# SAR-Research-Lab/lvt

Measured on AMD Instinct MI355X. Metric: stereo frames/sec (KITTI-shaped 1241x376), per-frame SE3 vs CPU ref, higher is better.
Workload: dtype u8/f64

## Files before the change

### include/lvt_amd_ext.h

```cpp
#ifndef LVT_AMD_EXT_H__
#define LVT_AMD_EXT_H__

#include "lvt_c.h"
#include <stdint.h>

#ifdef __cplusplus
extern "C" {
#endif

typedef struct lvt_amd_params {
    float fx, fy, cx, cy;
    float baseline;
    int img_width, img_height;
    float k1, k2, p1, p2, k3;
    float near_plane_distance, far_plane_distance;
    float triangulation_ratio_test_threshold;
    float tracking_ratio_test_threshold;
    float descriptor_matching_threshold;
    int min_num_matches_for_tracking;
    int tracking_radius;
    int detection_cell_size;
    int max_keypoints_per_cell;
    int agast_threshold;
    int untracked_threshold;
// ... 43 lines not shown
                                       unsigned *score, int score_cap, int counts[2]);

LVT_API void lvt_amd_set_stream(lvt_handle h, void *hip_stream);
LVT_API const char *lvt_amd_last_error(lvt_handle h);

LVT_API void lvt_amd_get_host_stats(lvt_handle h, long long out[8]);

LVT_API void lvt_amd_profile_enable(lvt_handle h, int enable);
LVT_API int lvt_amd_profile_read(lvt_handle h, int slot, char *name, int name_cap, double *total_ms, long *calls);

enum {
    LVT_AMD_C_N_LEFT = 0, LVT_AMD_C_N_RIGHT, LVT_AMD_C_MAP_SIZE, LVT_AMD_C_STAGED_SIZE, LVT_AMD_C_N_MATCHES,
    LVT_AMD_C_SECOND_PASS, LVT_AMD_C_N_ROW_MATCHES, LVT_AMD_C_N_TRIANGULATED, LVT_AMD_C_TRIANGULATED,
    LVT_AMD_C_RETRY_LEFT, LVT_AMD_C_RETRY_RIGHT, LVT_AMD_C_PNP_ITERS, LVT_AMD_C_PNP_INLIERS,
    LVT_AMD_C_MAP_SIZE_AT_MATCH, LVT_AMD_C_N_STAGED_ERASED, LVT_AMD_C_N_STAGED_PROMOTED, LVT_AMD_C_N_CULLED,
    LVT_AMD_C_FRAME, LVT_AMD_C_OVERFLOW ,
    LVT_AMD_C_PNP_BORDERLINE ,
    LVT_AMD_C_ROW_FALLBACK ,
    LVT_AMD_C_PNP_TRIALS , LVT_AMD_C_PNP_REJECTIONS ,
    LVT_AMD_C_PNP_TERMINATES ,
    LVT_AMD_C__COUNT = 32
};
LVT_API void lvt_amd_get_counts(lvt_handle h, int out[LVT_AMD_C__COUNT]);
LVT_API int lvt_amd_get_features(lvt_handle h, int eye, float *xy, float *resp, uint8_t *desc, int cap);
LVT_API int lvt_amd_get_matches(lvt_handle h, int *feat_idx, double *xyz, int cap);
LVT_API int lvt_amd_get_row_matches(lvt_handle h, int *pairs, int cap);
LVT_API int lvt_amd_get_map(lvt_handle h, double *xyz, int *counter, int *age, uint8_t *desc, int cap);
LVT_API int lvt_amd_get_staged(lvt_handle h, double *xyz, int *counter, uint8_t *desc, int cap);
LVT_API void lvt_amd_get_pose(lvt_handle h, double q_wxyz[4], double p[3]);
LVT_API int lvt_amd_get_last_pose(lvt_handle h, double q_wxyz[4], double p[3]);
LVT_API void lvt_amd_get_predicted_pose(lvt_handle h, double q_wxyz[4], double p[3]);
LVT_API void lvt_amd_get_debug(lvt_handle h, long long out[32]);
LVT_API void lvt_amd_get_timeline(lvt_handle h, long long out[16]);
LVT_API int lvt_amd_get_ordering(lvt_handle h);
LVT_API int lvt_amd_get_plane(lvt_handle h, int eye, int what, void *dst, int cap_bytes, int *pitch_out);

LVT_API int lvt_amd_pnp(const lvt_amd_params *p, const double q_in[4], const double p_in[3], const double *pts,
                        const float *obs, int n, double q_out[4], double p_out[3], int *n_solve_calls);
LVT_API int lvt_amd_pnp_detail(const lvt_amd_params *p, const double q_in[4], const double p_in[3], const double *pts,
                               const float *obs, int n, double q_out[4], double p_out[3], int *n_solve_calls,
                               double *err_out, int *level_out, int *borderline);
LVT_API int lvt_amd_pnp_trace(const lvt_amd_params *p, const double q_in[4], const double p_in[3], const double *pts,
                              const float *obs, int n, double q_out[4], double p_out[3], int *n_solve_calls,
                              double *err_out, int *level_out, int *borderline, double *trace, int trace_cap, int stats[3]);
LVT_API int lvt_amd_motion_predict(double state[14], const double q[4], const double p[3], double q_out[4], double p_out[3]);
LVT_API float lvt_amd_hamming_match_batched(const void *q_desc, const void *q_xy, const void *t_desc,
                                            const void *t_xy, const void *t_flag, int B, int M, int N,
                                            float r2, int mode, int img_rows, int img_cols, void *out,
                                            void *hip_stream);
LVT_API float lvt_amd_hamming_match_batched_n(const void *q_desc, const void *q_xy, const void *t_desc,
                                              const void *t_xy, const void *t_flag, int B, int M, int N,
                                              float r2, int mode, int img_rows, int img_cols, void *out,
                                              void *hip_stream, int launches);

typedef void *lvt_amd_rectifier;
LVT_API lvt_amd_rectifier lvt_amd_rectifier_create(const double K[9], const double D[5], const double R[9],
                                                   const double Pnew[9], int width, int height);
LVT_API void lvt_amd_rectifier_destroy(lvt_amd_rectifier r);
LVT_API int lvt_amd_rectify_device(lvt_amd_rectifier r, const void *d_src, int src_pitch, void *d_dst, int dst_pitch,
                                   void *hip_stream);
LVT_API int lvt_amd_rectify(lvt_amd_rectifier r, const unsigned char *src, unsigned char *dst);
LVT_API int lvt_amd_rectifier_get_maps(lvt_amd_rectifier r, float *map1, float *map2);
LVT_API int lvt_amd_set_rectifiers(lvt_handle h, lvt_amd_rectifier left, lvt_amd_rectifier right);
LVT_API int lvt_amd_batch_set_rectifiers(lvt_handle h, int seq, lvt_amd_rectifier left, lvt_amd_rectifier right);

enum { LVT_AMD_PIX_GRAY8 = 0, LVT_AMD_PIX_BGR8 = 1, LVT_AMD_PIX_RGB8 = 2, LVT_AMD_PIX_BGRA8 = 3, LVT_AMD_PIX_RGBA8 = 4 };
// ... 18 lines not shown
```

### lvt_amd/__init__.py

```python
from __future__ import annotations

import ctypes as C
import os

import numpy as np

from .params import LvtParameters, ParamsPOD, kitti_params, euroc_params, tum_params

_HERE = os.path.dirname(os.path.abspath(__file__))
LIB_PATH = os.environ.get("LVT_AMD_LIB") or os.path.join(_HERE, "lib", "liblvt_c.so")

ABI_SYMBOLS = [
    "lvt_create", "lvt_destroy", "lvt_track", "lvt_track_with_external_corners", "lvt_get_status",
    "lvt_amd_default_params", "lvt_amd_params_from_file", "lvt_amd_create", "lvt_amd_reset",
    "lvt_amd_track_rgbd", "lvt_amd_track_device", "lvt_amd_track_device_async", "lvt_amd_wait",
    "lvt_amd_set_stream", "lvt_amd_last_error", "lvt_amd_get_counts", "lvt_amd_get_features",
    "lvt_amd_get_matches", "lvt_amd_get_row_matches", "lvt_amd_get_map", "lvt_amd_get_staged",
    "lvt_amd_get_pose", "lvt_amd_get_last_pose", "lvt_amd_get_predicted_pose", "lvt_amd_get_plane", "lvt_amd_pnp", "lvt_amd_pnp_detail",
    "lvt_amd_hamming_match_batched", "lvt_amd_hamming_match_batched_n", "lvt_amd_rectifier_create", "lvt_amd_rectifier_destroy",
    "lvt_amd_rectify_device", "lvt_amd_rectify", "lvt_amd_rectifier_get_maps",
    "lvt_amd_odometry_create", "lvt_amd_odometry_destroy", "lvt_amd_odometry_reset", "lvt_amd_odometry_push_pose", "lvt_amd_odometry_update", "lvt_amd_profile_enable", "lvt_amd_profile_read", "lvt_amd_get_debug", "lvt_amd_get_timeline", "lvt_amd_get_ordering",
    "lvt_amd_batch_create", "lvt_amd_batch_size", "lvt_amd_batch_track_device_async", "lvt_amd_batch_wait",
    "lvt_amd_batch_get_counts", "lvt_amd_create_on_device", "lvt_amd_get_device", "lvt_amd_wait_status", "lvt_amd_get_host_stats",
    "lvt_amd_track_async", "lvt_amd_track_rgbd_async", "lvt_amd_pnp_trace", "lvt_amd_create_pooled", "lvt_amd_wait_pose",
    "lvt_amd_batch_create_mixed", "lvt_amd_batch_track_device_async_mixed", "lvt_amd_batch_get_params", "lvt_amd_batch_mixed_tables",
    "lvt_amd_track_rgbd_device", "lvt_amd_track_rgbd_device_async", "lvt_amd_track_rgbd16", "lvt_amd_track_rgbd16_async",
    "lvt_amd_batch_track_rgbd_device_async",
    "lvt_amd_set_rectifiers", "lvt_amd_batch_set_rectifiers",
    "lvt_amd_set_pixel_format", "lvt_amd_batch_set_pixel_format", "lvt_amd_get_pixel_format",
    "lvt_amd_motion_predict",
]

N_COUNTS = 32
COUNT_NAMES = ["n_left", "n_right", "map_size", "staged_size", "n_matches", "second_pass", "n_row_matches",
               "n_triangulated", "triangulated", "retry_left", "retry_right", "pnp_iters", "pnp_inliers",
               "map_size_at_match", "n_staged_erased", "n_staged_promoted", "n_culled", "frame", "overflow", "pnp_borderline", "row_fallback", "pnp_trials", "pnp_rejections", "pnp_terminates"]

eState_NOT_INITIALIZED, eState_TRACKING, eState_LOST = 1, 2, 3
eSensor_STEREO, eSensor_RGBD = 1, 2
PIX_GRAY8, PIX_BGR8, PIX_RGB8, PIX_BGRA8, PIX_RGBA8 = 0, 1, 2, 3, 4
PIX_BPP = {PIX_GRAY8: 1, PIX_BGR8: 3, PIX_RGB8: 3, PIX_BGRA8: 4, PIX_RGBA8: 4}
DEPTH_F32, DEPTH_U16 = 0, 1

_lib = None


def load_library():
    global _lib
    if _lib is not None:
        return _lib
    if not os.path.exists(LIB_PATH):
        raise RuntimeError(f"{LIB_PATH} is missing: build it with `make -C lvt_amd/csrc` "
                           "(there is no CPU fallback for the tracking path)")
    try:
        import torch
    except Exception:
        pass
    L = C.CDLL(LIB_PATH)
    vp = C.c_void_p
    L.lvt_create.restype = vp
    L.lvt_create.argtypes = [C.c_char_p, C.c_int]
    L.lvt_amd_create.restype = vp
    L.lvt_amd_create.argtypes = [vp, C.c_int]
# ... 12 lines not shown
    L.lvt_amd_track_rgbd.argtypes = [vp, vp, vp, C.c_int, C.c_int, vp, vp]
    L.lvt_amd_track_device.argtypes = [vp, vp, vp, C.c_int, C.c_int, C.c_int, vp, vp]
    L.lvt_amd_track_device_async.argtypes = [vp, vp, vp, C.c_int, C.c_int, C.c_int]
    L.lvt_amd_wait.argtypes = [vp, vp, vp]
    L.lvt_amd_track_async.argtypes = [vp, vp, vp, C.c_int, C.c_int]
    L.lvt_amd_track_async.restype = C.c_int
    L.lvt_amd_track_rgbd_async.argtypes = [vp, vp, vp, C.c_int, C.c_int]
    L.lvt_amd_track_rgbd_async.restype = C.c_int
    L.lvt_amd_wait_status.argtypes = [vp, vp, vp]
    L.lvt_amd_wait_status.restype = C.c_int
    L.lvt_amd_set_stream.argtypes = [vp, vp]
    L.lvt_amd_last_error.restype = C.c_char_p
    L.lvt_amd_last_error.argtypes = [vp]
    L.lvt_amd_get_counts.argtypes = [vp, vp]
    L.lvt_amd_get_features.argtypes = [vp, C.c_int, vp, vp, vp, C.c_int]
    L.lvt_amd_get_matches.argtypes = [vp, vp, vp, C.c_int]
    L.lvt_amd_get_row_matches.argtypes = [vp, vp, C.c_int]
    L.lvt_amd_get_map.argtypes = [vp, vp, vp, vp, vp, C.c_int]
    L.lvt_amd_get_staged.argtypes = [vp, vp, vp, vp, C.c_int]
    L.lvt_amd_get_pose.argtypes = [vp, vp, vp]
    L.lvt_amd_get_last_pose.argtypes = [vp, vp, vp]
    L.lvt_amd_get_predicted_pose.argtypes = [vp, vp, vp]
    L.lvt_amd_get_plane.argtypes = [vp, C.c_int, C.c_int, vp, C.c_int, vp]
    L.lvt_amd_pnp.argtypes = [vp, vp, vp, vp, vp, C.c_int, vp, vp, vp]
    L.lvt_amd_pnp_detail.argtypes = [vp, vp, vp, vp, vp, C.c_int, vp, vp, vp, vp, vp, vp]
    L.lvt_amd_pnp_trace.argtypes = [vp, vp, vp, vp, vp, C.c_int, vp, vp, vp, vp, vp, vp, vp, C.c_int, vp]
    L.lvt_amd_motion_predict.argtypes = [vp, vp, vp, vp, vp]
    L.lvt_amd_motion_predict.restype = C.c_int
    L.lvt_amd_hamming_match_batched.restype = C.c_float
    L.lvt_amd_hamming_match_batched.argtypes = [vp, vp, vp, vp, vp, C.c_int, C.c_int, C.c_int, C.c_float, C.c_int, C.c_int, C.c_int, vp, vp]
    L.lvt_amd_get_timeline.argtypes = [vp, vp]
    L.lvt_amd_get_ordering.argtypes = [vp]
    L.lvt_amd_get_ordering.restype = C.c_int
    L.lvt_amd_rectifier_create.restype = vp
    L.lvt_amd_rectifier_create.argtypes = [vp, vp, vp, vp, C.c_int, C.c_int]
    L.lvt_amd_rectifier_destroy.argtypes = [vp]
    L.lvt_amd_rectify_device.argtypes = [vp, vp, C.c_int, vp, C.c_int, vp]
    L.lvt_amd_rectify.argtypes = [vp, vp, vp]
    L.lvt_amd_rectifier_get_maps.argtypes = [vp, vp, vp]
    L.lvt_amd_odometry_create.restype = vp
    L.lvt_amd_odometry_create.argtypes = [vp, vp, C.c_int]
    L.lvt_amd_odometry_destroy.argtypes = [vp]
    L.lvt_amd_odometry_reset.argtypes = [vp]
    L.lvt_amd_odometry_push_pose.restype = C.c_int
    L.lvt_amd_odometry_push_pose.argtypes = [vp, vp, vp, C.c_int, C.c_double, vp, vp]
    L.lvt_amd_odometry_update.restype = C.c_int
    L.lvt_amd_odometry_update.argtypes = [vp, vp, vp, C.c_int, C.c_int, C.c_double, vp, vp]
    L.lvt_amd_hamming_match_batched_n.restype = C.c_float
    L.lvt_amd_hamming_match_batched_n.argtypes = [vp, vp, vp, vp, vp, C.c_int, C.c_int, C.c_int, C.c_float, C.c_int, C.c_int, C.c_int, vp, vp, C.c_int]
    L.lvt_amd_profile_enable.argtypes = [vp, C.c_int]
    L.lvt_amd_batch_create.restype = vp
    L.lvt_amd_batch_create.argtypes = [vp, C.c_int, C.c_int]
    L.lvt_amd_batch_size.argtypes = [vp]
    L.lvt_amd_batch_track_device_async.argtypes = [vp, vp, vp, C.c_int, C.c_int, C.c_int]
    L.lvt_amd_batch_wait.argtypes = [vp, vp, vp, vp]
    L.lvt_amd_batch_get_counts.argtypes = [vp, C.c_int, vp]
    L.lvt_amd_batch_create_mixed.restype = vp
    L.lvt_amd_batch_create_mixed.argtypes = [vp, C.c_int, C.c_int]
    L.lvt_amd_batch_track_device_async_mixed.restype = C.c_int
    L.lvt_amd_batch_track_device_async_mixed.argtypes = [vp, vp, vp, vp, vp, vp]
    L.lvt_amd_batch_get_params.restype = C.c_int
    L.lvt_amd_batch_get_params.argtypes = [vp, C.c_int, vp]
    L.lvt_amd_batch_mixed_tables.restype = C.c_int
    L.lvt_amd_batch_mixed_tables.argtypes = [vp, C.c_int, C.c_int, vp, C.c_int, vp, C.c_int, vp]
    L.lvt_amd_batch_size.restype = C.c_int
    for name, argtypes in (
# ... 515 lines not shown
```

### lvt_amd/csrc/k_track.hip

```cpp
#include "lvt_dev.h"
#include "wave_reduce.h"
#include "lvt_math.h"

namespace lvt {

enum : int { MODE_MAP = 0, MODE_STAGED = 1, MODE_ROW = 2 };

__device__ __forceinline__ void frame_prologue(const Seq &S, Ctl &c, int par, const Pose &predicted, const double mm_next[14], bool active,
                                               bool first, bool skipped) {
    const bool absent = skipped && S.fb[par].fc->absent != 0;
    if (!absent) {
        for (int i = 0; i < N_COUNTS; i++) c.counts[i] = 0;
        c.counts[C_FRAME] = c.frame_number;
        c.frame_number++;
    }
    c.active = active ? 1 : 0;
    c.first_frame = first ? 1 : 0;
    c.do_pass2 = 0;
    c.n_pass1 = c.n_pass2 = 0;
    c.n_matches = 0;
    c.lost_now = 0;
    c.need_tri = 0;
    c.dont_stage = 0;
    c.n_pairs = 0;
// ... 250 lines not shown
            for (int e = lane; e < cnt; e += 64) {
                const uint32_t k = buf[e];
                int rank = 0;
                for (int o = 0; o < cnt; o++) rank += (buf[o] < k) ? 1 : 0;
                cand[(size_t)i * KC + rank] = k;
            }
        }
        if (lane == 0) ncand[i] = cnt;
        __builtin_amdgcn_fence(__ATOMIC_ACQ_REL, "workgroup");
    }
}

template <int MODE, bool BV>
__global__ __launch_bounds__(256) void k_candidates(SeqArg<BV> sa, int pass2, int par, seq_t need_seq, int only_fb) {
    const Seq &S = sa.get();
    if (only_fb && !S.lists_fb[MODE == MODE_ROW ? 1 : 0]) return;
    if (MODE != MODE_ROW) {
        const Ctl &ctl = *S.ctl;
        if (!ctl.active || ctl.first_frame) return;
        if (MODE == MODE_STAGED && (ctl.lost_now || S.prm.staged_th <= 0)) return;
    } else {
        if (S.prm.sensor != 1) return;
        if (need_seq && __hip_atomic_load(&S.fb[par].fc->feat_seq, __ATOMIC_ACQUIRE, __HIP_MEMORY_SCOPE_AGENT) < need_seq) return;
    }
    __shared__ uint32_t lbuf[4 * KC];
    __shared__ float s_tx[NF_MAX], s_ty[NF_MAX];
    __shared__ uint32_t s_tc[NF_MAX];
    CandLds C;
    C.lbuf = lbuf, C.tx = s_tx, C.ty = s_ty, C.tc = s_tc;
    candidates_body<MODE>(S, pass2, par, C, blockIdx.x * 4 + wave_id(), gridDim.x * 4, 256);
}

__device__ __forceinline__ void deliver_record(const Ctl &ctl, Ctl *rec_out, seq_t *done_out, seq_t seq, int nthreads);
__device__ __forceinline__ void gate_late_poll(Ctl &ctl, FeatCtl &fc, seq_t seq);
template <bool BV>
__global__ __launch_bounds__(256) void k_match_map(SeqArg<BV> sa, int par, seq_t seq, int gated, Ctl *prev_rec, seq_t *prev_done) {
    const Seq &S = sa.get();
    Ctl &ctl = *S.ctl;
    __shared__ int s_state;
    if (gated) {
        if (threadIdx.x == 0 && blockIdx.x == 0) ctl.dbg[38] = (long long)wall_clock64();
        if (blockIdx.x == 0 && prev_rec) deliver_record(ctl, prev_rec, prev_done, seq - 1, 256);
        if (threadIdx.x == 0) {
            if (blockIdx.x == 0) {
                gate_late_poll(ctl, *S.fb[par].fc, seq);
                __hip_atomic_store(&ctl.late_gate_seq, seq, __ATOMIC_RELEASE, __HIP_MEMORY_SCOPE_AGENT);
            } else {
                while (__hip_atomic_load(&ctl.late_gate_seq, __ATOMIC_ACQUIRE, __HIP_MEMORY_SCOPE_AGENT) < seq) __builtin_amdgcn_s_sleep(8);
            }
        }
    }
    if (threadIdx.x == 0 && blockIdx.x == 0) ctl.dbg[40] = (long long)wall_clock64();
    __shared__ int s_skip;
    if (threadIdx.x == 0) {
        int sk = ctl.skip;
        if (!gated && __hip_atomic_load(&S.fb[par].fc->skip_seq, __ATOMIC_ACQUIRE, __HIP_MEMORY_SCOPE_AGENT) == seq) {
            sk = 1;
            if (blockIdx.x == 0) ctl.skip = 1;
        }
        s_state = ctl.state, s_skip = sk;
    }
    __syncthreads();
    const int state = s_state;
    const bool skipped = s_skip != 0;
    const bool active = (state != 3) && !skipped, first = (state == 1);
    __shared__ double w2c[12];
    if (threadIdx.x == 0) {
        Pose predicted;
        double mmn[14];
        if (active && !first) {
            motion_predict(ctl, ctl.last_pose, predicted, mmn);
            world_to_camera(predicted, w2c);
        }
        if (blockIdx.x == 0) {
            frame_prologue(S, ctl, par, predicted, mmn, active, first, skipped);
            if (active && !first) ctl.counts[C_MAP_SIZE_AT_MATCH] = *S.map_n;
        }
    }
    if (!active || first) return;
    __shared__ uint32_t lbuf[4 * KC];
    __shared__ float s_tx[NF_MAX], s_ty[NF_MAX];
    __shared__ uint32_t s_tc[NF_MAX];
    CandLds C;
    C.lbuf = lbuf, C.tx = s_tx, C.ty = s_ty, C.tc = s_tc, C.w2c = w2c;
    candidates_body<MODE_MAP, true>(S, 0, par, C, blockIdx.x * 4 + wave_id(), gridDim.x * 4, 256, (ctl.early_ran_seq == seq) ? max(ctl.early_done, 0) : 0, -1);
}

__device__ __forceinline__ void gate_buf_wait(const Seq &S, seq_t want, int par) {
    Ctl &ctl = *S.ctl;
    const unsigned long long t0 = wall_clock64();
    while (__hip_atomic_load(&ctl.track_done_seq, __ATOMIC_ACQUIRE, __HIP_MEMORY_SCOPE_AGENT) < want) {
        __builtin_amdgcn_s_sleep(8);
        if (wall_clock64() - t0 > 200000000ull) {
            S.fb[par].fc->poison = 1;
            atomicAdd(&ctl.gate_fatal, 1);
            __threadfence();
            break;
        }
    }
}
__global__ __launch_bounds__(64) void k_gate_buf(const Seq *seqs, seq_t want, int par) {
    if (threadIdx.x != 0) return;
    gate_buf_wait(seq_const(seqs, blockIdx.z), want, par);
}

__global__ void k_feat_done(const Seq *seqs, int par, seq_t seq) {
    if (threadIdx.x != 0) return;
    FeatCtl &fc = *seq_const(seqs, blockIdx.x).fb[par].fc;
    seq_const(seqs, blockIdx.x).ctl->dbg[47] = (long long)wall_clock64();
    if (fc.poison) {
        fc.skip_seq = seq;
        fc.poison = 0;
    }
    __threadfence();
    atomicExch(&fc.feat_seq, seq);
}

__global__ void k_row_done(const Seq *seqs, int par, seq_t seq) {
    if (threadIdx.x != 0) return;
    FeatCtl &fc = *seq_const(seqs, blockIdx.x).fb[par].fc;
    if (__hip_atomic_load(&fc.feat_seq, __ATOMIC_ACQUIRE, __HIP_MEMORY_SCOPE_AGENT) < seq) return;
    __threadfence();
    atomicExch(&fc.row_seq, seq);
}

template <bool BV>
__global__ __launch_bounds__(64) void k_gate(SeqArg<BV> sa, int par, seq_t want, seq_t seq, int test_timeout) {
    if (threadIdx.x == 0 && blockIdx.x == 0) sa.get().ctl->dbg[32] = (long long)wall_clock64();
    Ctl &ctl = *sa.get().ctl;
    FeatCtl &fc = *sa.get().fb[par].fc;
    if (threadIdx.x != 0) return;
    bool ok = true;
    if (test_timeout) {
        atomicAdd(&ctl.gate_timeouts, 1);
        ok = false;
    } else {
        const unsigned long long t0 = wall_clock64();
        while (__hip_atomic_load(&fc.feat_seq, __ATOMIC_ACQUIRE, __HIP_MEMORY_SCOPE_AGENT) < seq) {
            __builtin_amdgcn_s_sleep(8);
            if (wall_clock64() - t0 > 2000000ull) {
                atomicAdd(&ctl.gate_timeouts, 1);
                ok = false;
                break;
            }
        }
        if (ok && __hip_atomic_load(&fc.skip_seq, __ATOMIC_ACQUIRE, __HIP_MEMORY_SCOPE_AGENT) == seq) ok = false;
        const unsigned long long t1 = wall_clock64();
        ctl.dbg[35] = (long long)t1;
        while (ok && __hip_atomic_load(&ctl.pnp_seq, __ATOMIC_ACQUIRE, __HIP_MEMORY_SCOPE_AGENT) < want) {
            __builtin_amdgcn_s_sleep(8);
            if (wall_clock64() - t1 > 2000000ull) {
                atomicAdd(&ctl.gate_timeouts, 1);
                ok = false;
                break;
            }
        }
    }
    const seq_t mine = 4u * seq + (ok ? 1u : 3u);
    seq_t cur = __hip_atomic_load(&ctl.early_state, __ATOMIC_ACQUIRE, __HIP_MEMORY_SCOPE_AGENT);
    for (;;) {
        if (cur >= 4u * seq + 1u) {
            ok = false;
            break;
        }
        const seq_t seen = atomicCAS(&ctl.early_state, cur, mine);
        if (seen == cur) break;
        cur = seen;
    }
    ctl.gate_ok = ok ? seq : (seq_t)0;
    ctl.dbg[33] = (long long)wall_clock64();
}

template <bool BV>
__global__ __launch_bounds__(256) void k_early_map(SeqArg<BV> sa, int par, seq_t seq, int only_fb) {
    if (threadIdx.x == 0 && blockIdx.x == 0) sa.get().ctl->dbg[34] = (long long)wall_clock64();
    const Seq &S = sa.get();
    if (only_fb && !S.lists_fb[0]) return;
    Ctl &ctl = *S.ctl;
    const int n_early = (ctl.gate_ok == seq) ? ctl.early_done : 0;
    if (n_early <= 0) return;
    __shared__ double w2c[12];
    if (threadIdx.x == 0) {
        Pose predicted;
        double mmn[14];
        motion_predict(ctl, ctl.last_pose, predicted, mmn);
        world_to_camera(predicted, w2c);
    }
    __shared__ uint32_t lbuf[4 * KC];
    __shared__ float s_tx[NF_MAX], s_ty[NF_MAX];
// ... 629 lines not shown
        {
            CandLds C;
            C.lbuf = r_lists;
            C.tx = reinterpret_cast<float *>(r_lists + 16 * KC);
            C.ty = C.tx + NF_MAX;
            C.tc = reinterpret_cast<uint32_t *>(C.ty + NF_MAX);
            candidates_body<MODE_MAP>(S, 1, par, C, wave_id(), RES_THREADS / 64, RES_THREADS);
        }
        __syncthreads();
        resolve_body<MODE_MAP>(S, ctl, 1, par, L, r_tab);
        __syncthreads();
    }
    if (*S.map_n <= RES_THREADS) {
        bookkeep_cull_small(S, ctl, par, L.scan);
        return;
    }
    bookkeep_cull_large(S, ctl, par, L.scan, L.lists);
}

template <bool BV>
__global__ __launch_bounds__(RES_THREADS) void k_early_mid(SeqArg<BV> sa, int par, seq_t seq) {
    if (threadIdx.x == 0 && blockIdx.x == 0) sa.get().ctl->dbg[36] = (long long)wall_clock64();
    const Seq &S = sa.get();
    Ctl &ctl = *S.ctl;
    const int n_early = (ctl.gate_ok == seq) ? ctl.early_done : 0;
    if (n_early > 0) {
        RESOLVE_LDS_DECL
        resolve_body<MODE_MAP>(S, ctl, 0, par, L, r_tab, 1, n_early);
        __syncthreads();
        if (threadIdx.x == 0) ctl.early_ran_seq = seq;
    }
    if (threadIdx.x == 0) {
        ctl.dbg[37] = (long long)wall_clock64();
        __threadfence();
        if (n_early > 0 || ctl.gate_ok == seq) atomicCAS(&ctl.early_state, 4u * seq + 1u, 4u * seq + 2u);
    }
}

__device__ __forceinline__ void deliver_record(const Ctl &ctl, Ctl *rec_out, seq_t *done_out, seq_t seq, int nthreads) {
    static_assert(sizeof(Ctl) % 8 == 0, "record copy");
    const unsigned long long *src = reinterpret_cast<const unsigned long long *>(&ctl);
    unsigned long long *dst = reinterpret_cast<unsigned long long *>(rec_out);
    for (int i = threadIdx.x; i < (int)(sizeof(Ctl) / 8); i += nthreads) dst[i] = __hip_atomic_load(&src[i], __ATOMIC_RELAXED, __HIP_MEMORY_SCOPE_AGENT);
    __threadfence_system();
    __syncthreads();
    if (threadIdx.x == 0) __hip_atomic_store(done_out, seq, __ATOMIC_RELEASE, __HIP_MEMORY_SCOPE_SYSTEM);
}
__global__ __launch_bounds__(64) void k_deliver(const Seq *seqs, Ctl *rec_out, seq_t *done_out, seq_t seq) {
    deliver_record(*seq_const(seqs, blockIdx.z).ctl, rec_out + blockIdx.z, done_out + blockIdx.z, seq, 64);
}

__device__ __forceinline__ void gate_late_poll(Ctl &ctl, FeatCtl &fc, seq_t seq) {
    unsigned long long t0 = wall_clock64();
    for (;;) {
        const seq_t cur = __hip_atomic_load(&ctl.early_state, __ATOMIC_ACQUIRE, __HIP_MEMORY_SCOPE_AGENT);
        if (cur >= 4u * seq + 2u) break;
        __builtin_amdgcn_s_sleep(8);
        if (wall_clock64() - t0 > 6000000ull) {
            atomicAdd(&ctl.gate_timeouts, 1);
            if (cur < 4u * seq + 1u && atomicCAS(&ctl.early_state, cur, 4u * seq + 3u) == cur) break;
            t0 = wall_clock64();
        }
    }
    t0 = wall_clock64();
    while (__hip_atomic_load(&fc.feat_seq, __ATOMIC_ACQUIRE, __HIP_MEMORY_SCOPE_AGENT) < seq) {
        __builtin_amdgcn_s_sleep(8);
        if (wall_clock64() - t0 > 200000000ull) {
            ctl.skip = 1;
            atomicAdd(&ctl.gate_fatal, 1);
            break;
        }
    }
    if (__hip_atomic_load(&fc.skip_seq, __ATOMIC_ACQUIRE, __HIP_MEMORY_SCOPE_AGENT) == seq) ctl.skip = 1;
}

template <bool BV>
__global__ __launch_bounds__(64) void k_gate_late(SeqArg<BV> sa, int par, seq_t seq, Ctl *prev_rec, seq_t *prev_done) {
    if (threadIdx.x == 0 && blockIdx.x == 0) sa.get().ctl->dbg[38] = (long long)wall_clock64();
    Ctl &ctl = *sa.get().ctl;
    FeatCtl &fc = *sa.get().fb[par].fc;
    if (prev_rec) deliver_record(ctl, prev_rec + blockIdx.z, prev_done + blockIdx.z, seq - 1, 64);
    if (threadIdx.x == 0) gate_late_poll(ctl, fc, seq);
}

__device__ __forceinline__ double rcp_nr(double s) {
    double y = __builtin_amdgcn_rcp(s);
#pragma unroll
    for (int it = 0; it < 2; it++) y = __builtin_fma(__builtin_fma(-s, y, 1.0), y, y);
    return y;
}
__device__ __forceinline__ double log_ge1(double a) {
    int e = __builtin_amdgcn_frexp_exp(a);
    double m = __builtin_amdgcn_frexp_mant(a);
    const bool lo = m < 0.70710678118654752440;
    m = lo ? m + m : m;
    e = lo ? e - 1 : e;
    const double s = (m - 1.0) * rcp_nr(m + 1.0);
    const double z = s * s;
    double p = 1.0 / 21.0;
    p = __builtin_fma(p, z, 1.0 / 19.0);
    p = __builtin_fma(p, z, 1.0 / 17.0);
    p = __builtin_fma(p, z, 1.0 / 15.0);
    p = __builtin_fma(p, z, 1.0 / 13.0);
    p = __builtin_fma(p, z, 1.0 / 11.0);
    p = __builtin_fma(p, z, 1.0 / 9.0);
    p = __builtin_fma(p, z, 1.0 / 7.0);
// ... 883 lines not shown
```

### lvt_amd/csrc/lvt_dev.h

```cpp
#pragma once
#include <hip/hip_runtime.h>
#include <stdint.h>

namespace lvt {

constexpr int NF_MAX = 4096;
constexpr int CELLS_MAX = 64;
constexpr int CELL_OUT_CAP = 2048;
constexpr int RAW_CAP = 10240;
constexpr int CELL_SIDE_LDS = 1024;
constexpr int CELL_SIDE_MAX = 4096;
constexpr int BIG_CELL_SIDE = 256;
constexpr int MAP_MAX = 32768;
constexpr int STAGED_MAX = 16384;
constexpr int KC = 128;
constexpr int N_COUNTS = 32;

enum : int { OVF_RAW = 1, OVF_CELL_OUT = 2, OVF_FEATURES = 4, OVF_MAP = 8, OVF_STAGED = 16, OVF_CELL_DIM = 32 };

enum : int {
    C_N_LEFT = 0, C_N_RIGHT, C_MAP_SIZE, C_STAGED_SIZE, C_N_MATCHES, C_SECOND_PASS, C_N_ROW_MATCHES,
    C_N_TRIANGULATED, C_TRIANGULATED, C_RETRY_LEFT, C_RETRY_RIGHT, C_PNP_ITERS, C_PNP_INLIERS,
    C_MAP_SIZE_AT_MATCH, C_N_STAGED_ERASED, C_N_STAGED_PROMOTED, C_N_CULLED, C_FRAME, C_OVERFLOW, C_PNP_BORDERLINE,
    C_ROW_FALLBACK,
// ... 16 lines not shown
    float min_x, max_x, min_y, max_y;
    int W, H;
    int min_matches, tracking_radius, cell_size, max_kp_cell, agast_th, agast_th_low;
    int untracked_th, staged_th, tri_policy;
    int cells_x, cells_y, n_cells;
    int hash_ccx, hash_ccy, cell_search_radius;
    int sensor;
    int undistort;
    unsigned cell_magic;
    int big_cell_strips;
};

struct Pose {
    double q[4];
    double p[3];
};

using seq_t = unsigned long long;

struct Ctl {
    int state;
    int frame_number;
    int last_matches[3];
    Pose last_pose;
    double mm_last_q[4], mm_ang_vel[4], mm_last_p[3], mm_lin_vel[3];
    double mm_next[14];
    int mm_pending;
    int early_done;
    int early_accepted;
    seq_t pnp_seq, gate_ok, early_ran_seq;
    seq_t early_state;
    seq_t track_done_seq;
    seq_t late_gate_seq;
    int gate_timeouts;
    int gate_fatal;
    int skip;
    int active;
    int first_frame;
    int do_pass2;
    int n_pass1, n_pass2;
    int n_matches;
    int lost_now;
    int need_tri;
    int dont_stage;
    int n_pairs;
    Pose predicted, optimized;
    int counts[N_COUNTS];
    int overflow;
    long long dbg[48];
    double out_R[9], out_t[3];
    int out_status;
};

constexpr int NPAR = 3;

enum { DEPTH_F32 = 0, DEPTH_U16 = 1 };

struct FrameIn {
    const uint8_t *img[2];
    const float *depth_img;
    int img_pitch, depth_pitch;
    int depth_format;
    float depth_scale;
    const float *ext_xy[2];
};

// ... 141 lines not shown
```

### lvt_amd/csrc/lvt_host.hip

```cpp
#define LVT_EXPORT_FUNCTIONS
#include "../../include/lvt_amd_ext.h"

#include "k_features.hip"
#include "k_track.hip"
#include "k_hamming.hip"
#include "k_lists.hip"
#include "k_rectify.hip"
#include "lvt_odometry.h"

#include <atomic>
#include <cmath>
#include <chrono>
#include <cstdio>
#include <cstdlib>
#include <cstring>
#include <string>
#include <functional>
#include <vector>

namespace lvt {

#define HIPCHK(ctx, call)                                                                  \
    do {                                                                                   \
        hipError_t e__ = (call);                                                           \
// ... 52 lines not shown
    if (t0 < n - tail0) dst[tail0 + t0] = src[tail0 + t0];
}
static void launch_stage_copy(hipStream_t st, const uint8_t *src, float *d_dst, size_t n, int fmt) {
    if (fmt == DEPTH_U16) hipLaunchKernelGGL(k_stage_copy<uint16_t>, dim3(256), dim3(256), 0, st, reinterpret_cast<const uint16_t *>(src), reinterpret_cast<uint16_t *>(d_dst), n);
    else hipLaunchKernelGGL(k_stage_copy<float>, dim3(256), dim3(256), 0, st, reinterpret_cast<const float *>(src), d_dst, n);
}

constexpr int MAX_DEVICES = 64;
static std::atomic<int> g_live_contexts[MAX_DEVICES];

constexpr uint64_t CTX_MAGIC = 0x4C56545F43545831ull, SLOT_MAGIC = 0x4C56545F534C5431ull;

struct Rectifier {
    int w = 0, h = 0, pitch = 0;
    int device = 0;
    float *d_map1 = nullptr, *d_map2 = nullptr;
    int2 *d_fix = nullptr;
    uint8_t *d_src = nullptr, *d_dst = nullptr;
};

struct HostStage {
    uint8_t *h = nullptr, *dev = nullptr;
    size_t second = 0;
};

struct Context {
    uint64_t magic = CTX_MAGIC;
    double host_enq_us = 0, host_wait_us = 0;
    long host_enq_n = 0, host_wait_n = 0;
    int gate_timeouts_seen = 0, gate_fatal_seen = 0;
    bool want_events = false, ordering_forced = false;
    hipEvent_t ev_switch = nullptr, ev_switch_e = nullptr;
    long test_gate_timeout = 0, switched_at = -1;
    long long planes_in_place = 0, planes_staged = 0;
    int device = 0;
    int B = 1;
    int launch_seqs = 0;
    int ring_seqs[8] = {};
    int sensor = 1;
    Params prm{};
    bool mixed = false;
    std::vector<Params> prms;
    std::vector<lvt_amd_params> in_prms;
    uint32_t *d_score_tab = nullptr, *d_cells_tab = nullptr;
    int n_score_wgs = 0, n_cells_wgs = 0;
    bool any_staged = false, any_strips = false;
    int max_cells = 0;
    const Params &seq_prm(int s) const { return mixed ? prms[s] : prm; }
    hipStream_t stream = nullptr;
    hipStream_t stream_f = nullptr;
    hipStream_t stream_e = nullptr;
    bool own_stream = false;
    std::vector<void *> allocs;
    const Seq *d_seqs = nullptr;
    std::vector<Seq> h_seqs;
    std::vector<Ctl *> d_ctl;
    Ctl *h_ctl = nullptr;
    Ctl *h_ctl_dev = nullptr;
    seq_t *h_done = nullptr, *h_done_dev = nullptr;
    PoseRec *h_pose = nullptr, *h_pose_dev = nullptr;
    seq_t *h_pose_done = nullptr, *h_pose_done_dev = nullptr;
    bool binned_lists = false;
    bool early_pose = true;
    bool early_pending = false;
    FrameArgs *h_fargs = nullptr;
    hipEvent_t ev_done[RING] = {};
// ... 346 lines not shown
        c->prm = prm;
        c->mixed = mixed;
        if (mixed) c->prms = prms;
        c->in_prms.assign(in, in + prms.size());
        for (const Params &q : prms) {
            c->any_staged = c->any_staged || q.staged_th > 0;
            c->any_strips = c->any_strips || q.big_cell_strips != 0;
            c->max_cells = std::max(c->max_cells, q.n_cells);
        }
        HIPCHK(c, hipStreamCreateWithFlags(&c->stream, hipStreamNonBlocking));
        {
            int ncu = 0;
            if (B >= 2 && B <= 28) {
                int total = 0;
                if (hipDeviceGetAttribute(&total, hipDeviceAttributeMultiprocessorCount, device) == hipSuccess && total >= 64) ncu = total / 8 * 7;
            }
            if (const char *e = std::getenv("LVT_AMD_FEATURE_CUS")) ncu = (B >= 2) ? std::atoi(e) : 0;
            if (ncu > 0 && ncu < 1024) {
                uint32_t mask[32] = {};
                for (int i = 0; i < ncu; i++) mask[i >> 5] |= 1u << (i & 31);
                HIPCHK(c, hipExtStreamCreateWithCUMask(&c->stream_f, 32, mask));
                c->feature_cus = ncu;
            } else
                HIPCHK(c, hipStreamCreateWithFlags(&c->stream_f, hipStreamNonBlocking));
        }
        HIPCHK(c, hipStreamCreateWithFlags(&c->stream_e, hipStreamNonBlocking));
        c->own_stream = true;
        for (auto &e : c->ev_done) HIPCHK(c, hipEventCreateWithFlags(&e, hipEventDisableTiming));
        for (auto &e : c->ev_feat) HIPCHK(c, hipEventCreateWithFlags(&e, hipEventDisableTiming));
        HIPCHK(c, hipEventCreateWithFlags(&c->ev_depth, hipEventDisableTiming));
        HIPCHK(c, hipEventCreateWithFlags(&c->ev_switch, hipEventDisableTiming));
        HIPCHK(c, hipEventCreateWithFlags(&c->ev_switch_e, hipEventDisableTiming));
        if (const char *e = std::getenv("LVT_AMD_TEST_GATE_TIMEOUT")) c->test_gate_timeout = std::atol(e);
        {
            const char *o = std::getenv("LVT_AMD_ORDERING");
            if (o && std::strcmp(o, "events") == 0) c->events_only = true;
            else if (o && std::strcmp(o, "polling") == 0) c->events_only = false, c->ordering_forced = true;
            else c->events_only = B == 1 && c->live_on_device() > 1;
        }
        c->pitch = ((prm.W + 63) / 64) * 64;
        HIPCHK(c, hipHostMalloc((void **)&c->h_ctl, sizeof(Ctl) * B * RING, hipHostMallocCoherent));
        HIPCHK(c, hipHostGetDevicePointer((void **)&c->h_ctl_dev, c->h_ctl, 0));
        HIPCHK(c, hipHostMalloc((void **)&c->h_done, sizeof(seq_t) * B * RING, hipHostMallocCoherent));
        HIPCHK(c, hipHostGetDevicePointer((void **)&c->h_done_dev, c->h_done, 0));
        std::memset(c->h_done, 0, sizeof(seq_t) * B * RING);
        HIPCHK(c, hipHostMalloc((void **)&c->h_pose, sizeof(PoseRec) * B * RING, hipHostMallocCoherent));
        HIPCHK(c, hipHostGetDevicePointer((void **)&c->h_pose_dev, c->h_pose, 0));
        HIPCHK(c, hipHostMalloc((void **)&c->h_pose_done, sizeof(seq_t) * B * RING, hipHostMallocCoherent));
        HIPCHK(c, hipHostGetDevicePointer((void **)&c->h_pose_done_dev, c->h_pose_done, 0));
        std::memset(c->h_pose_done, 0, sizeof(seq_t) * B * RING);
        if (const char *e = std::getenv("LVT_AMD_SYNC_TAIL")) c->early_pose = std::strcmp(e, "wait") != 0;
        c->binned_lists = B > 1;
        if (const char *e = std::getenv("LVT_AMD_BINNED_LISTS")) c->binned_lists = std::atoi(e) != 0;
        if (const char *e = std::getenv("LVT_AMD_TEST_ROW_FALLBACK")) c->force_row_fallback = std::atoi(e) != 0;
        {
            int idx[CELLS_MAX], area[CELLS_MAX];
            for (int cc = 0; cc < prm.n_cells; cc++) {
                const int cx = cc % prm.cells_x, cy = cc / prm.cells_x;
                idx[cc] = cc;
                area[cc] = std::min(prm.cell_size, prm.W - cx * prm.cell_size) * std::min(prm.cell_size, prm.H - cy * prm.cell_size);
            }
            std::stable_sort(idx, idx + prm.n_cells, [&](int a, int b) { return area[a] > area[b]; });
            for (int cc = 0; cc < CELLS_MAX; cc++) c->cell_order.v[cc] = (uint8_t)(cc < prm.n_cells ? idx[cc] : 0);
        }
        if (std::getenv("LVT_AMD_NO_FEAT_PACK")) c->feat_pack = false;
        if (const char *e = std::getenv("LVT_AMD_BRIEF_FROM_IMAGE")) c->brief_from_image = std::atoi(e) ? 1 : 0;
// ... 348 lines not shown
    if (c->brief_from_image) LAUNCH_S(6, sf, k_brief_img, dim3(64, 2, Bz), dim3(256), 0, par, brief_publishes ? (seq_t)(c->enq + 1) : (seq_t)0);
    else LAUNCH_S(6, sf, k_brief, dim3(64, 2, Bz), dim3(256), 0, par, brief_publishes ? (seq_t)(c->enq + 1) : (seq_t)0);
    if (!evo && !brief_publishes) hipLaunchKernelGGL(k_feat_done, dim3(Bz), dim3(64), 0, sf, S, par, (seq_t)(c->enq + 1));
    const int bl = c->binned_lists ? 1 : 0;
    if (evo && bl && c->sensor == 1) LAUNCH_SM(19, sf, k_hamming_batched_lists, MODE_ROW, dim3(c->lists_wgs_row, 1, Bz), dim3(LS_THREADS), LS_LDS_BYTES, par, (seq_t)0);
    if (evo) LAUNCH_SM(18, sf, k_candidates, MODE_ROW, dim3(256, 1, Bz), dim3(256), 0, 0, par, (seq_t)0, bl);
    if (evo) hipLaunchKernelGGL(k_feat_done, dim3(Bz), dim3(64), 0, sf, S, par, (seq_t)(c->enq + 1));
    if (evo) (void)hipEventRecord(c->ev_feat[par], sf);
    const seq_t seq = (seq_t)(c->enq + 1);
    if (!evo) {
        hipStream_t se = c->stream_e;
        LAUNCH_S(1, se, k_gate, dim3(1, 1, Bz), dim3(64), 0, par, (seq_t)c->enq, seq, (c->test_gate_timeout && (long)seq == c->test_gate_timeout) ? 1 : 0);
        if (bl) LAUNCH_SM(11, se, k_hamming_batched_lists, MODE_MAP, dim3(c->lists_wgs_map, 1, Bz), dim3(LS_THREADS), LS_LDS_BYTES, par, seq);
        LAUNCH_S(9, se, k_early_map, dim3((bl && B > 1) ? 32 : 256, 1, Bz), dim3(256), 0, par, seq, bl);
        LAUNCH_S(10, se, k_early_mid, dim3(1, 1, Bz), dim3(RES_THREADS), 0, par, seq);
        if (c->sensor == 1) {
            if (bl) LAUNCH_SM(19, se, k_hamming_batched_lists, MODE_ROW, dim3(c->lists_wgs_row, 1, Bz), dim3(LS_THREADS), LS_LDS_BYTES, par, seq);
            LAUNCH_SM(18, se, k_candidates, MODE_ROW, dim3(B == 1 ? ROW_BLOCKS : ROW_BLOCKS_BATCH, 1, Bz), dim3(256), 0, 0, par, seq, bl);
            hipLaunchKernelGGL(k_row_done, dim3(Bz), dim3(64), 0, se, S, par, seq);
        }
    }
    {
        Ctl *prec = nullptr;
        seq_t *pdone = nullptr;
        if (!evo && c->delivered < c->enq) {
            const int pslot = (int)((c->enq - 1) % RING);
            prec = c->h_ctl_dev + (size_t)pslot * B, pdone = c->h_done_dev + (size_t)pslot * B;
            c->delivered = c->enq;
        }
        if (evo) {
            (void)hipStreamWaitEvent(st, c->ev_feat[par], 0);
            LAUNCH_S(8, st, k_match_map, dim3(256, 1, Bz), dim3(256), 0, par, seq, 0, (Ctl *)nullptr, (seq_t *)nullptr);
        } else if (B == 1 && c->live_on_device() <= MAX_FOLDED_GATES) {
            LAUNCH_S(8, st, k_match_map, dim3(MATCH_BLOCKS_GATED, 1, 1), dim3(256), 0, par, seq, 1, prec, pdone);
        } else {
            LAUNCH_S(7, st, k_gate_late, dim3(1, 1, Bz), dim3(64), 0, par, seq, prec, pdone);
            LAUNCH_S(8, st, k_match_map, dim3(B > 1 ? c->match_blocks_batch : 256, 1, Bz), dim3(256), 0, par, seq, 0, (Ctl *)nullptr, (seq_t *)nullptr);
        }
    }
    LAUNCH_S(12, st, k_track_mid, dim3(1, 1, Bz), dim3(RES_THREADS), 0, par, seq);
    {
        const bool ep = c->sync_call && c->early_pose && !c->prof && B == 1;
        LAUNCH_S(13, st, k_pnp, dim3(1, 1, Bz), dim3(PNP_THREADS), PNP_DYN_BYTES, par, seq, ep ? c->h_pose_dev + (size_t)slot * B : (PoseRec *)nullptr,
                 ep ? c->h_pose_done_dev + (size_t)slot * B : (seq_t *)nullptr);
    }
    if (c->any_staged)
        LAUNCH_SM(16, st, k_candidates, MODE_STAGED, dim3(64, 1, Bz), dim3(256), 0, 0, par, (seq_t)0, 0);
    LAUNCH_S(20, st, k_triangulate, dim3(1, 1, Bz), dim3(1024), 0, par, seq, c->h_ctl_dev + (size_t)slot * B,
           c->h_done_dev + (size_t)slot * B, evo ? 0 : (c->force_row_fallback ? 2 : 1), (evo || c->sync_call) ? 1 : 0);
    if (evo || c->sync_call) c->delivered = c->enq + 1;
    if (evo) (void)hipEventRecord(c->ev_done[slot], st);
    c->enq++;
}

static void collect_oldest(Context *c) {
    HostTimer ht(&c->host_wait_us);
    c->host_wait_n++;
    if (c->done >= c->enq) return;
    const int slot = (int)(c->done % RING);
    const int Bz = (c->ring_seqs[slot] > 0 && c->ring_seqs[slot] <= c->B) ? c->ring_seqs[slot] : c->B;
    if (c->delivered < c->done + 1) {
        hipLaunchKernelGGL(k_deliver, dim3(1, 1, Bz), dim3(64), 0, c->stream, c->d_seqs, c->h_ctl_dev + (size_t)slot * c->B,
                           c->h_done_dev + (size_t)slot * c->B, (seq_t)(c->done + 1));
        c->delivered = c->done + 1;
    }
    {
        const seq_t want = (seq_t)(c->done + 1);
// ... 1232 lines not shown
    return -1;
}
LVT_API void lvt_amd_get_pose(lvt_handle h, double q[4], double p[3]) {
    h = resolve_handle(h);
    try {
        View v;
        if (!view_of(h, v)) return;
        for (int k = 0; k < 4; k++) q[k] = v.rec->last_pose.q[k];
        for (int k = 0; k < 3; k++) p[k] = v.rec->last_pose.p[k];
    } catch (...) {
    }
}
LVT_API void lvt_amd_get_predicted_pose(lvt_handle h, double q[4], double p[3]) {
    h = resolve_handle(h);
    try {
        View v;
        if (!view_of(h, v)) return;
        for (int k = 0; k < 4; k++) q[k] = v.rec->predicted.q[k];
        for (int k = 0; k < 3; k++) p[k] = v.rec->predicted.p[k];
    } catch (...) {
    }
}
LVT_API void lvt_amd_get_debug(lvt_handle h, long long out[32]) {
    h = resolve_handle(h);
    if (!is_ctx(h)) return;
    Context *c = static_cast<Context *>(h);
    DeviceGuard guard(c);
    try {
        drain(c);
        for (int i = 0; i < 32; i++) out[i] = last_ctl(c).dbg[i];
    } catch (...) {
    }
}
LVT_API int lvt_amd_get_ordering(lvt_handle h) {
    if (is_auto(h)) {
        AutoHandle *A = static_cast<AutoHandle *>(h);
        std::lock_guard<std::mutex> g(A->mu);
        return lvt_amd_get_ordering(A->impl);
    }
    if (is_slot(h)) return 2;
    return h && static_cast<Context *>(h)->events_only ? 1 : 0;
}
LVT_API void lvt_amd_get_timeline(lvt_handle h, long long out[16]) {
    h = resolve_handle(h);
    if (!is_ctx(h)) return;
    Context *c = static_cast<Context *>(h);
    DeviceGuard guard(c);
    try {
        if (c->early_pending) drain(c);
    } catch (...) {
    }
    for (int i = 0; i < 16; i++) out[i] = last_ctl(c).dbg[32 + i];
}
LVT_API int lvt_amd_get_plane(lvt_handle h, int eye, int what, void *dst, int cap_bytes, int *pitch_out) {
    h = resolve_handle(h);
    if (!is_ctx(h)) return -1;
    Context *c = static_cast<Context *>(h);
    DeviceGuard guard(c);
    try {
        drain(c);
        const FrameBuf &FB = c->h_seqs[0].fb[c->last_par];
        const size_t n = (size_t)c->pitch * c->prm.H;
        if (what == 2) {
            if (!c->has_rect(0) || c->done == 0) return 0;
            if ((size_t)cap_bytes < n) return -1;
            HIPCHK(c, hipMemcpy(dst, c->d_rect[(size_t)c->last_par * 2 + (eye ? 1 : 0)], n, hipMemcpyDeviceToHost));
// ... 439 lines not shown
```

Baseline: 8831.

## Deliver previous frame record via dedicated courier workgroup in gated match kernel

Adds an extra workgroup to the gated k_match_map launch that copies the previous frame's control record to host-visible memory in parallel, using one register per thread. The first-block serial copy is removed from the gate's critical path, and a rec_taken handshake makes the gate wait for the snapshot before the Ctl state is mutated. Several spin-wait polls also switch from acquire loads to relaxed loads followed by a single acquire fence, which cuts per-iteration fence cost. The added handshake brings a risk of ordering bugs and a possible extra wait on the gate path.

```diff
diff --git a/include/lvt_amd_ext.h b/include/lvt_amd_ext.h
--- a/include/lvt_amd_ext.h
+++ b/include/lvt_amd_ext.h
@@ -99,6 +99,7 @@
 LVT_API void lvt_amd_get_predicted_pose(lvt_handle h, double q_wxyz[4], double p[3]);
 LVT_API void lvt_amd_get_debug(lvt_handle h, long long out[32]);
 LVT_API void lvt_amd_get_timeline(lvt_handle h, long long out[16]);
+LVT_API int lvt_amd_get_record_counts(lvt_handle h, int out[LVT_AMD_C__COUNT]);
 LVT_API int lvt_amd_get_ordering(lvt_handle h);
 LVT_API int lvt_amd_get_plane(lvt_handle h, int eye, int what, void *dst, int cap_bytes, int *pitch_out);
 
diff --git a/lvt_amd/__init__.py b/lvt_amd/__init__.py
--- a/lvt_amd/__init__.py
+++ b/lvt_amd/__init__.py
@@ -28,7 +28,7 @@
     "lvt_amd_batch_track_rgbd_device_async",
     "lvt_amd_set_rectifiers", "lvt_amd_batch_set_rectifiers",
     "lvt_amd_set_pixel_format", "lvt_amd_batch_set_pixel_format", "lvt_amd_get_pixel_format",
-    "lvt_amd_motion_predict",
+    "lvt_amd_motion_predict", "lvt_amd_get_record_counts",
 ]
 
 N_COUNTS = 32
@@ -107,6 +107,8 @@
     L.lvt_amd_get_timeline.argtypes = [vp, vp]
     L.lvt_amd_get_ordering.argtypes = [vp]
     L.lvt_amd_get_ordering.restype = C.c_int
+    L.lvt_amd_get_record_counts.argtypes = [vp, vp]
+    L.lvt_amd_get_record_counts.restype = C.c_int
     L.lvt_amd_rectifier_create.restype = vp
     L.lvt_amd_rectifier_create.argtypes = [vp, vp, vp, vp, C.c_int, C.c_int]
     L.lvt_amd_rectifier_destroy.argtypes = [vp]
diff --git a/lvt_amd/csrc/k_track.hip b/lvt_amd/csrc/k_track.hip
--- a/lvt_amd/csrc/k_track.hip
+++ b/lvt_amd/csrc/k_track.hip
@@ -306,21 +306,31 @@
 }
 
 __device__ __forceinline__ void deliver_record(const Ctl &ctl, Ctl *rec_out, seq_t *done_out, seq_t seq, int nthreads);
-__device__ __forceinline__ void gate_late_poll(Ctl &ctl, FeatCtl &fc, seq_t seq);
+__device__ __forceinline__ void courier_deliver(Ctl &ctl, Ctl *rec_out, seq_t *done_out, seq_t seq);
+__device__ __forceinline__ void record_taken_wait(Ctl &ctl, Ctl *rec_out, seq_t *done_out, seq_t seq);
+__device__ __forceinline__ void gate_late_poll(Ctl &ctl, FeatCtl &fc, seq_t seq, Ctl *courier_rec = nullptr, seq_t *courier_done = nullptr);
 template <bool BV>
 __global__ __launch_bounds__(256) void k_match_map(SeqArg<BV> sa, int par, seq_t seq, int gated, Ctl *prev_rec, seq_t *prev_done) {
     const Seq &S = sa.get();
     Ctl &ctl = *S.ctl;
     __shared__ int s_state;
+    const bool courier = gated == 2 && prev_rec;
+    const int n_wgs = (int)gridDim.x - (courier ? 1 : 0);
+    if (courier && (int)blockIdx.x == n_wgs) {
+        courier_deliver(ctl, prev_rec, prev_done, seq);
+        return;
+    }
     if (gated) {
-        if (threadIdx.x == 0 && blockIdx.x == 0) ctl.dbg[38] = (long long)wall_clock64();
-        if (blockIdx.x == 0 && prev_rec) deliver_record(ctl, prev_rec, prev_done, seq - 1, 256);
+        const long long t_start = (long long)wall_clock64();
+        if (blockIdx.x == 0 && prev_rec && !courier) deliver_record(ctl, prev_rec, prev_done, seq - 1, 256);
         if (threadIdx.x == 0) {
             if (blockIdx.x == 0) {
-                gate_late_poll(ctl, *S.fb[par].fc, seq);
+                gate_late_poll(ctl, *S.fb[par].fc, seq, courier ? prev_rec : nullptr, prev_done);
+                ctl.dbg[38] = t_start;
                 __hip_atomic_store(&ctl.late_gate_seq, seq, __ATOMIC_RELEASE, __HIP_MEMORY_SCOPE_AGENT);
             } else {
-                while (__hip_atomic_load(&ctl.late_gate_seq, __ATOMIC_ACQUIRE, __HIP_MEMORY_SCOPE_AGENT) < seq) __builtin_amdgcn_s_sleep(8);
+                while (__hip_atomic_load(&ctl.late_gate_seq, __ATOMIC_RELAXED, __HIP_MEMORY_SCOPE_AGENT) < seq) __builtin_amdgcn_s_sleep(8);
+                __builtin_amdgcn_fence(__ATOMIC_ACQUIRE, "agent");
             }
         }
     }
@@ -357,7 +367,7 @@
     __shared__ uint32_t s_tc[NF_MAX];
     CandLds C;
     C.lbuf = lbuf, C.tx = s_tx, C.ty = s_ty, C.tc = s_tc, C.w2c = w2c;
-    candidates_body<MODE_MAP, true>(S, 0, par, C, blockIdx.x * 4 + wave_id(), gridDim.x * 4, 256, (ctl.early_ran_seq == seq) ? max(ctl.early_done, 0) : 0, -1);
+    candidates_body<MODE_MAP, true>(S, 0, par, C, blockIdx.x * 4 + wave_id(), n_wgs * 4, 256, (ctl.early_ran_seq == seq) ? max(ctl.early_done, 0) : 0, -1);
 }
 
 __device__ __forceinline__ void gate_buf_wait(const Seq &S, seq_t want, int par) {
@@ -410,7 +420,7 @@
         ok = false;
     } else {
         const unsigned long long t0 = wall_clock64();
-        while (__hip_atomic_load(&fc.feat_seq, __ATOMIC_ACQUIRE, __HIP_MEMORY_SCOPE_AGENT) < seq) {
+        while (__hip_atomic_load(&fc.feat_seq, __ATOMIC_RELAXED, __HIP_MEMORY_SCOPE_AGENT) < seq) {
             __builtin_amdgcn_s_sleep(8);
             if (wall_clock64() - t0 > 2000000ull) {
                 atomicAdd(&ctl.gate_timeouts, 1);
@@ -418,10 +428,10 @@
                 break;
             }
         }
-        if (ok && __hip_atomic_load(&fc.skip_seq, __ATOMIC_ACQUIRE, __HIP_MEMORY_SCOPE_AGENT) == seq) ok = false;
+        if (ok && __hip_atomic_load(&fc.skip_seq, __ATOMIC_RELAXED, __HIP_MEMORY_SCOPE_AGENT) == seq) ok = false;
         const unsigned long long t1 = wall_clock64();
         ctl.dbg[35] = (long long)t1;
-        while (ok && __hip_atomic_load(&ctl.pnp_seq, __ATOMIC_ACQUIRE, __HIP_MEMORY_SCOPE_AGENT) < want) {
+        while (ok && __hip_atomic_load(&ctl.pnp_seq, __ATOMIC_RELAXED, __HIP_MEMORY_SCOPE_AGENT) < want) {
             __builtin_amdgcn_s_sleep(8);
             if (wall_clock64() - t1 > 2000000ull) {
                 atomicAdd(&ctl.gate_timeouts, 1);
@@ -429,6 +439,7 @@
                 break;
             }
         }
+        __builtin_amdgcn_fence(__ATOMIC_ACQUIRE, "agent");
     }
     const seq_t mine = 4u * seq + (ok ? 1u : 3u);
     seq_t cur = __hip_atomic_load(&ctl.early_state, __ATOMIC_ACQUIRE, __HIP_MEMORY_SCOPE_AGENT);
@@ -1124,7 +1135,8 @@
     }
     if (threadIdx.x == 0) {
         ctl.dbg[37] = (long long)wall_clock64();
-        __threadfence();
+        __builtin_amdgcn_fence(__ATOMIC_RELEASE, "agent");
+        asm volatile("s_waitcnt vmcnt(0)" ::: "memory");
         if (n_early > 0 || ctl.gate_ok == seq) atomicCAS(&ctl.early_state, 4u * seq + 1u, 4u * seq + 2u);
     }
 }
@@ -1142,28 +1154,77 @@
     deliver_record(*seq_const(seqs, blockIdx.z).ctl, rec_out + blockIdx.z, done_out + blockIdx.z, seq, 64);
 }
 
-__device__ __forceinline__ void gate_late_poll(Ctl &ctl, FeatCtl &fc, seq_t seq) {
+__device__ __forceinline__ void courier_deliver(Ctl &ctl, Ctl *rec_out, seq_t *done_out, seq_t seq) {
+    constexpr int WORDS = (int)(sizeof(Ctl) / 8);
+    static_assert(sizeof(Ctl) % 8 == 0 && WORDS <= 256, "the courier holds the record in one register per thread");
+    __shared__ int s_mine;
+    if (threadIdx.x == 0) s_mine = (atomicMax(&ctl.rec_taken, 2u * seq) < 2u * seq) ? 1 : 0;
+    __syncthreads();
+    if (!s_mine) return;
+    const unsigned long long *src = reinterpret_cast<const unsigned long long *>(&ctl);
+    unsigned long long *dst = reinterpret_cast<unsigned long long *>(rec_out);
+    const int i = threadIdx.x;
+    unsigned long long v = 0;
+    if (i < WORDS) v = __hip_atomic_load(&src[i], __ATOMIC_RELAXED, __HIP_MEMORY_SCOPE_AGENT);
+    asm volatile("s_waitcnt vmcnt(0)" ::: "memory");
+    __syncthreads();
+    if (i == 0) __hip_atomic_store(&ctl.rec_taken, 2u * seq + 1u, __ATOMIC_RELEASE, __HIP_MEMORY_SCOPE_AGENT);
+    if (i < WORDS) dst[i] = v;
+    __threadfence_system();
+    __syncthreads();
+    if (i == 0) __hip_atomic_store(done_out, seq - 1, __ATOMIC_RELEASE, __HIP_MEMORY_SCOPE_SYSTEM);
+}
+__device__ __forceinline__ void record_taken_wait(Ctl &ctl, Ctl *rec_out, seq_t *done_out, seq_t seq) {
     unsigned long long t0 = wall_clock64();
+    while (__hip_atomic_load(&ctl.rec_taken, __ATOMIC_RELAXED, __HIP_MEMORY_SCOPE_AGENT) < 2u * seq + 1u) {
+        __builtin_amdgcn_s_sleep(2);
+        if (wall_clock64() - t0 > 2000000ull) {
+            if (atomicMax(&ctl.rec_taken, 2u * seq) < 2u * seq) {
+                const unsigned long long *src = reinterpret_cast<const unsigned long long *>(&ctl);
+                unsigned long long *dst = reinterpret_cast<unsigned long long *>(rec_out);
+                for (int i = 0; i < (int)(sizeof(Ctl) / 8); i++) dst[i] = __hip_atomic_load(&src[i], __ATOMIC_RELAXED, __HIP_MEMORY_SCOPE_AGENT);
+                __threadfence_system();
+                __hip_atomic_store(done_out, seq - 1, __ATOMIC_RELEASE, __HIP_MEMORY_SCOPE_SYSTEM);
+                __hip_atomic_store(&ctl.rec_taken, 2u * seq + 1u, __ATOMIC_RELEASE, __HIP_MEMORY_SCOPE_AGENT);
+                break;
+            }
+            t0 = wall_clock64();
+        }
+    }
+}
+
+__device__ __forceinline__ void gate_late_poll(Ctl &ctl, FeatCtl &fc, seq_t seq, Ctl *courier_rec, seq_t *courier_done) {
+    unsigned long long t0 = wall_clock64();
+    seq_t cur;
     for (;;) {
-        const seq_t cur = __hip_atomic_load(&ctl.early_state, __ATOMIC_ACQUIRE, __HIP_MEMORY_SCOPE_AGENT);
+        cur = __hip_atomic_load(&ctl.early_state, __ATOMIC_RELAXED, __HIP_MEMORY_SCOPE_AGENT);
         if (cur >= 4u * seq + 2u) break;
         __builtin_amdgcn_s_sleep(8);
         if (wall_clock64() - t0 > 6000000ull) {
+            if (courier_rec) record_taken_wait(ctl, courier_rec, courier_done, seq);
             atomicAdd(&ctl.gate_timeouts, 1);
             if (cur < 4u * seq + 1u && atomicCAS(&ctl.early_state, cur, 4u * seq + 3u) == cur) break;
             t0 = wall_clock64();
         }
     }
-    t0 = wall_clock64();
-    while (__hip_atomic_load(&fc.feat_seq, __ATOMIC_ACQUIRE, __HIP_MEMORY_SCOPE_AGENT) < seq) {
-        __builtin_amdgcn_s_sleep(8);
-        if (wall_clock64() - t0 > 200000000ull) {
+    if (cur != 4u * seq + 2u) {
+        t0 = wall_clock64();
+        while (__hip_atomic_load(&fc.feat_seq, __ATOMIC_RELAXED, __HIP_MEMORY_SCOPE_AGENT) < seq) {
+            __builtin_amdgcn_s_sleep(8);
+            if (wall_clock64() - t0 > 200000000ull) {
+                if (courier_rec) record_taken_wait(ctl, courier_rec, courier_done, seq);
+                ctl.skip = 1;
+                atomicAdd(&ctl.gate_fatal, 1);
+                break;
+            }
+        }
+        if (__hip_atomic_load(&fc.skip_seq, __ATOMIC_RELAXED, __HIP_MEMORY_SCOPE_AGENT) == seq) {
+            if (courier_rec) record_taken_wait(ctl, courier_rec, courier_done, seq);
             ctl.skip = 1;
-            atomicAdd(&ctl.gate_fatal, 1);
-            break;
-        }
-    }
-    if (__hip_atomic_load(&fc.skip_seq, __ATOMIC_ACQUIRE, __HIP_MEMORY_SCOPE_AGENT) == seq) ctl.skip = 1;
+        }
+    }
+    if (courier_rec) record_taken_wait(ctl, courier_rec, courier_done, seq);
+    __builtin_amdgcn_fence(__ATOMIC_ACQUIRE, "agent");
 }
 
 template <bool BV>
diff --git a/lvt_amd/csrc/lvt_dev.h b/lvt_amd/csrc/lvt_dev.h
--- a/lvt_amd/csrc/lvt_dev.h
+++ b/lvt_amd/csrc/lvt_dev.h
@@ -72,6 +72,7 @@
     seq_t early_state;
     seq_t track_done_seq;
     seq_t late_gate_seq;
+    seq_t rec_taken;
     int gate_timeouts;
     int gate_fatal;
     int skip;
diff --git a/lvt_amd/csrc/lvt_host.hip b/lvt_amd/csrc/lvt_host.hip
--- a/lvt_amd/csrc/lvt_host.hip
+++ b/lvt_amd/csrc/lvt_host.hip
@@ -108,6 +108,7 @@
     bool want_events = false, ordering_forced = false;
     hipEvent_t ev_switch = nullptr, ev_switch_e = nullptr;
     long test_gate_timeout = 0, switched_at = -1;
+    bool record_courier = true;
     long long planes_in_place = 0, planes_staged = 0;
     int device = 0;
     int B = 1;
@@ -520,6 +521,7 @@
         HIPCHK(c, hipEventCreateWithFlags(&c->ev_switch, hipEventDisableTiming));
         HIPCHK(c, hipEventCreateWithFlags(&c->ev_switch_e, hipEventDisableTiming));
         if (const char *e = std::getenv("LVT_AMD_TEST_GATE_TIMEOUT")) c->test_gate_timeout = std::atol(e);
+        if (const char *e = std::getenv("LVT_AMD_RECORD_COURIER")) c->record_courier = std::atoi(e) != 0;
         {
             const char *o = std::getenv("LVT_AMD_ORDERING");
             if (o && std::strcmp(o, "events") == 0) c->events_only = true;
@@ -934,7 +936,8 @@
             (void)hipStreamWaitEvent(st, c->ev_feat[par], 0);
             LAUNCH_S(8, st, k_match_map, dim3(256, 1, Bz), dim3(256), 0, par, seq, 0, (Ctl *)nullptr, (seq_t *)nullptr);
         } else if (B == 1 && c->live_on_device() <= MAX_FOLDED_GATES) {
-            LAUNCH_S(8, st, k_match_map, dim3(MATCH_BLOCKS_GATED, 1, 1), dim3(256), 0, par, seq, 1, prec, pdone);
+            const int cour = (prec && c->record_courier) ? 1 : 0;
+            LAUNCH_S(8, st, k_match_map, dim3(MATCH_BLOCKS_GATED + cour, 1, 1), dim3(256), 0, par, seq, 1 + cour, prec, pdone);
         } else {
             LAUNCH_S(7, st, k_gate_late, dim3(1, 1, Bz), dim3(64), 0, par, seq, prec, pdone);
             LAUNCH_S(8, st, k_match_map, dim3(B > 1 ? c->match_blocks_batch : 256, 1, Bz), dim3(256), 0, par, seq, 0, (Ctl *)nullptr, (seq_t *)nullptr);
@@ -2233,6 +2236,23 @@
     } catch (...) {
     }
 }
+LVT_API int lvt_amd_get_record_counts(lvt_handle h, int out[LVT_AMD_C__COUNT]) {
+    h = resolve_handle(h);
+    if (!is_ctx(h)) return -1;
+    Context *c = static_cast<Context *>(h);
+    DeviceGuard guard(c);
+    try {
+        if (c->early_pending) drain(c);
+    } catch (...) {
+        return -1;
+    }
+    if (c->B != 1 || c->done <= 0) return -1;
+    const Ctl &r = last_ctl(c);
+    if (out)
+        for (int i = 0; i < LVT_AMD_C__COUNT; i++) out[i] = r.counts[i];
+    return r.rec_taken == 2u * (seq_t)(c->done + 1) ? 1 : 0;
+}
+
 LVT_API int lvt_amd_get_ordering(lvt_handle h) {
     if (is_auto(h)) {
         AutoHandle *A = static_cast<AutoHandle *>(h);
```

Result: slower. 8433 (-4.5%).
